# Reecepbcups/celestia-app

Hardware: AMD Instinct MI355X
Metric: ODS→EDS+DAH blocks/sec at k=128 (1/8 GPU); achieved HBM GB/s (higher is better)
Workload: dtype u8; 1 GPU; k128_block_batch: da.ExtendShares+NewDataAvailabilityHeader on 128 independent k=128 blocks per GPU per step (configs[1] per block, batched as configs[2]); k=128, parallelism=blocks x1

## Files before the change

### celestia-app_amd/csrc/cda_internal.h

```cpp
#pragma once
#include <hip/hip_runtime.h>
#include <stddef.h>
#include <stdint.h>

#include "../../include/cda.h"

#define CDA_SHARE 512
#define CDA_REC_WORDS 24
#define CDA_REC_BYTES 96

#ifndef CDA_TEST_HOOKS
#define CDA_TEST_HOOKS 0
#endif
#if CDA_TEST_HOOKS
#define CDA_AB_ENV(name) getenv(name)
#else
#define CDA_AB_ENV(name) ((const char*)nullptr)
#endif

namespace cda {

struct LeoTables {
  int bits;
  unsigned order, modulus;
  const uint16_t* exp_t;
  const uint16_t* log_t;
  const uint16_t* skew;
};
const LeoTables& leo_tables(int bits);
uint64_t leo8_colbits(unsigned log_m);
void leo16_colbits(unsigned log_m, uint16_t out[16]);

struct RsJob {
  const uint8_t* src;
  long long src_blk, src_cw, src_sh;
  uint8_t* dst;
  long long dst_blk, dst_cw, dst_sh;
  uint8_t* cpy;
  long long cpy_blk, cpy_cw, cpy_sh;
  int k;
  int cw_per_blk;
  int nblk;
  int shard_len;
};

int rs_init_device_tables(int device);
int rs16_init_device_tables(int device);
int rs_decode_init_device_tables(int device);
int launch_rs_decode(uint8_t* d_base, const long long* d_off, const long long* d_stride, const uint8_t* d_present,
                     int ncw, int k, int shard_len, hipStream_t s);
int launch_rs_encode8(const RsJob& job, hipStream_t s);
bool rs8_reg_batched(const RsJob& job);
int launch_rs_encode8_pair(const RsJob& ja, const RsJob& jb, bool remap, hipStream_t s);
int launch_q0_copy(const uint8_t* d_ods, uint8_t* d_eds, int k, int nblocks, int max_wgs, hipStream_t s);
int launch_rs_encode16(const RsJob& job, hipStream_t s);
bool rs16_reg_eligible(const RsJob& j);
const char* rs16_diag_tag();
const char* rs8_diag_tag();
int rs16_reg_init(int device);
int launch_rs_encode16_reg(const RsJob& j, const uint16_t* d_cpoly, hipStream_t s);
int launch_leaf_hash(const uint8_t* d_eds, void* d_leaf_nodes, unsigned long long* d_status, int k, int nblocks,
                     hipStream_t s, const uint8_t* d_ods = nullptr);
int launch_nmt_level(const void* d_in, void* d_out, bool from_leaves, int k, int nblocks, int level, hipStream_t s);
int launch_nmt_trees(const void* d_leaves, void* d_levels, void* d_roots, int k, int nblocks, hipStream_t s,
                     void* prof_ctx, bool l1_quads = true);
int launch_dah(const void* d_roots, void* d_dah, int n_roots_total, int nblocks, hipStream_t s);
int launch_dah_tree(const void* d_roots, void* d_dah, void* d_nodes_out, int n_roots_total, hipStream_t s);
int launch_dah_wide(const void* d_roots, void* d_dah, unsigned* d_done, void* d_digests, int n, int nblocks,
                    hipStream_t s);
int launch_trees_lds(const void* d_leaves, void* d_roots, void* d_dah, unsigned* d_done, void* d_digests, int k,
                     int nblocks, hipStream_t s);
int launch_axis_leaf(const uint8_t* d_leaves, int n, uint64_t square_size, uint64_t axis_index, void* d_nodes,
                     unsigned long long* d_status, hipStream_t s);
int launch_level_generic(const void* d_in, void* d_out, int n_in, hipStream_t s);
constexpr int kAxisRootsMaxLeaves = 1024;
int launch_axis_roots(const uint8_t* d_leaves, long long tree_stride, int n, uint64_t square_size,
                      const unsigned long long* d_axis_idx, int ntrees, void* d_roots, unsigned long long* d_status,
                      hipStream_t s);
int launch_axes_roots(const uint8_t* d_eds, int k, const int* d_axes, int axis0, int ntrees, int leaf_off, int nleaves,
                      void* d_nodes, void* d_scratch, void* d_roots, unsigned long long* d_status, hipStream_t s);
int launch_nmt_fold(void* d_nodes, void* d_scratch, void* d_roots, int ntrees, int log2n, hipStream_t s);
int launch_parity_compare(const uint8_t* d_eds, int k, const int* d_axes, int naxes, const uint8_t* d_par,
                          unsigned* d_flags, hipStream_t s);
int launch_axes_verify(const uint8_t* d_eds, int k, const int* d_axes, int ntrees, const uint8_t* d_want_rows,
                       const uint8_t* d_want_cols, unsigned* d_flag, unsigned base, bool per_tree, hipStream_t s);
int launch_roots_check(const void* d_recs, const unsigned long long* d_status, const int* d_axes, int n,
                       const uint8_t* d_want_rows, const uint8_t* d_want_cols, unsigned* d_flag, unsigned base,
                       hipStream_t s);

struct BlobDesc {
  unsigned long long data_off;
  uint32_t len;
  uint32_t share_off;
  uint32_t nshares;
  uint32_t width;
  uint8_t ns[32];
};
int launch_blob_shares(const BlobDesc* d_desc, int nblobs, const uint8_t* d_data, uint32_t total, uint8_t* d_shares,
                       hipStream_t s);
int launch_blob_leaves(const uint8_t* d_shares, uint32_t total, void* d_recs, hipStream_t s);
int launch_blob_mountain_level(const BlobDesc* d_desc, int nblobs, void* d_recs, uint32_t total, int level,
                               hipStream_t s);
int launch_pack_tree_level(const void* d_recs, void* d_out, int log2w, int h, bool col, uint32_t t0, uint32_t nt,
                           uint32_t off_h, hipStream_t s);
int launch_merkle_sets(const void* d_recs, const uint32_t* d_idx, const uint32_t* d_off, int nsets, int max_set,
                       void* d_out, void* d_nodes_out, hipStream_t s);

int launch_scatter_cell_runs(const void* d_compact, void* d_dst, const uint32_t* d_dst_cell, const uint32_t* d_pre,
                             int nruns, uint32_t ncells, hipStream_t s, bool same_layout = false);
int launch_build_ods(const cda_share_segment* d_segs, int nseg, const uint8_t* d_data, const uint32_t* d_reserved,
                     uint32_t nshares, void* d_ods, hipStream_t s);

struct TreeSpec {
  const void* leaves;
  unsigned long long t_stride, i_stride;
  uint32_t ntrees;
  bool tree_fastest;
  void* scratch;
  void* roots;
  unsigned long long r_stride;
};

inline int raise_dynamic_lds(const void* kernel, size_t bytes) {
  if (bytes <= 64 * 1024) return 0;
  return hipFuncSetAttribute(kernel, hipFuncAttributeMaxDynamicSharedMemorySize, (int)bytes) == hipSuccess ? 0 : -1;
}

struct SubtreeLaunch {
  int M, log2n_out;
};
inline SubtreeLaunch subtree_launch(int L, int l_in) {
  const int rest = L - l_in;
  const int M = rest == 3 ? 3 : (rest < 2 ? rest : 2);
  return {M, rest - M};
}
inline unsigned long long levels_before(unsigned long long trees, int L, int l) {
// ... 16 lines not shown
```

### celestia-app_amd/csrc/ctx.h

```cpp
#pragma once
#include <hip/hip_runtime.h>

#include <map>
#include <mutex>
#include <string>
#include <thread>
#include <vector>

#include "arena.h"
#include "cda_internal.h"
#include "mixed_route.h"

namespace cda {
struct AxisQueue;
struct Stager;
struct Consensus;
}
struct cda_square;

struct cda_ctx {
  int device = 0;
  std::vector<int> local_cpus;
  std::recursive_mutex mu;
  hipStream_t stream = nullptr;
  bool repair_overlap = true;
  bool repair_fused_verify = true;
  bool repair_early = true;
  bool l1_quads = true;
  int rs_sched = 2;
  size_t rs_min_ods_bytes = (size_t)256 << 20;
  bool rs_q3_cols = false;
  bool rs_pair_remap = false;
  int q0_copy_wgs = 64;
  hipStream_t q0_stream = nullptr;
  hipEvent_t q0_fork_ev = nullptr, q0_join_ev = nullptr;
  hipStream_t aux_stream = nullptr;
  hipEvent_t ws_event = nullptr, sync_ev = nullptr;
  bool ws_pending = false;
  static constexpr int kSlots = 3;
  hipStream_t h2d_stream = nullptr, d2h_stream = nullptr;
  hipEvent_t ev_h2d[kSlots] = {}, ev_comp[kSlots] = {}, ev_d2h[kSlots] = {};
  static constexpr int kJoin = 2;
  hipEvent_t fork_ev = nullptr, join_ev[kJoin] = {};
  std::string last_err;
  struct Buf {
    void* p = nullptr;
    size_t cap = 0;
  };
  Buf ods, eds, leaf, scratch, roots, dah, status, plan, payload;
  Buf done;
  Buf nodes;
  std::vector<cda_square*> squares;
  Buf sp_ods, sp_R, sp_LR, sp_S, sp_C, sp_LC, sp_scratch, sp_meta, sp_gather;
  hipEvent_t sp_ev[2] = {};
  Buf rdesc, rstage;
  Buf rcompact, rruns;
  cda::Stager* st_in = nullptr;
  cda::Stager* st_out = nullptr;
  int staging = 3;
  cda::Consensus* cons = nullptr;
  bool consensus = true;
  int cons_in = 0, cons_out = 0, cons_stg_mib = -1, copy_threads = 7;
  bool cons_trace = false;
  bool huge_pages = false;
  int mixed_small_max = cda::kMixedSmallMaxDefault;
  cda::AxisQueue* axq = nullptr;
  bool prof = false;
  struct Pending {
    std::string name;
    hipEvent_t a, b;
  };
  std::vector<Pending> pending;
  std::vector<hipEvent_t> event_pool;
  std::map<std::string, std::pair<double, long long>> prof_acc;
};

namespace cda {

constexpr uint32_t kMaxDeviceK = 512;
constexpr int kLdsTreesMax = 512;

bool dev_ok(cda_ctx* c, hipError_t e, const char* what);
int ensure(cda_ctx* c, cda_ctx::Buf& b, size_t bytes);
void flush_profile(cda_ctx* c);
struct Stage {
  cda_ctx* c;
  hipStream_t s;
  Arena ar;
  bool ok = true;
  template <class T>
  T* stage(const T* src, size_t count) {
    T* at = ar.take<T>(count);
    if (ok && at && count && !dev_ok(c, hipMemcpyAsync(at, src, count * sizeof(T), hipMemcpyHostToDevice, s), "H2D"))
      ok = false;
    return at;
  }
};
template <class Lay>
size_t staged_bytes(Lay& lay) {
  Stage measure{nullptr, nullptr, Arena()};
  lay(measure);
  return measure.ar.used();
}
inline bool copy_any(cda_ctx* c, void* dst, const void* src, size_t n, hipStream_t s) {
  return n == 0 || dev_ok(c, hipMemcpyAsync(dst, src, n, hipMemcpyDefault, s), "copy");
}
inline int verdicts_back(cda_ctx* c, void* dst, const void* d_src, size_t n, hipStream_t s) {
  if (!dev_ok(c, hipMemcpyAsync(dst, d_src, n, hipMemcpyDeviceToHost, s), "D2H") ||
      !dev_ok(c, hipStreamSynchronize(s), "sync"))
    return CDA_E_DEVICE;
  flush_profile(c);
  return CDA_OK;
}
int ilog2i(uint32_t v);
bool is_pow2(uint64_t v);
// ... 111 lines not shown
```

### celestia-app_amd/csrc/engine.cpp

```cpp
#include <hip/hip_runtime.h>

#include <algorithm>
#include <chrono>
#include <cmath>
#include <cstdlib>
#include <cstdio>
#include <cstring>
#include <map>
#include <mutex>
#include <string>
#include <system_error>
#include <thread>
#include <vector>

#include "ctx.h"
#include "small_square.h"

namespace cda {

ProfScope::ProfScope(void* c, const char* n, hipStream_t s) : ctx(c), name(n), stream(s), a(nullptr), b(nullptr) {
  cda_ctx* x = static_cast<cda_ctx*>(ctx);
  if (!x || !x->prof) return;
  auto get = [&]() {
    hipEvent_t e;
// ... 121 lines not shown
  j.cpy_cw = j.dst_cw;
  j.cpy_sh = S;
  j.k = (int)k;
  j.cw_per_blk = (int)k;
  j.nblk = (int)nblocks;
  j.shard_len = CDA_SHARE;
  return j;
}

RsJob cols_job(uint32_t k, uint32_t nblocks, uint8_t* d_eds) {
  const uint32_t w = 2 * k;
  const long long S = CDA_SHARE;
  RsJob j{};
  j.src = d_eds;
  j.src_blk = (long long)w * w * S;
  j.src_cw = S;
  j.src_sh = (long long)w * S;
  j.dst = d_eds + (size_t)k * w * S;
  j.dst_blk = j.src_blk;
  j.dst_cw = S;
  j.dst_sh = (long long)w * S;
  j.cpy = nullptr;
  j.k = (int)k;
  j.cw_per_blk = (int)w;
  j.nblk = (int)nblocks;
  j.shard_len = CDA_SHARE;
  return j;
}

int enqueue_rs(cda_ctx* c, uint32_t k, uint32_t nblocks, const uint8_t* d_ods, uint8_t* d_eds, hipStream_t s) {
  {
    const RsJob j = rows_job(k, nblocks, d_ods, d_eds);
    ProfScope ps(c, 2 * k <= 256 ? "rs_encode8_rows" : "rs_encode16_rows", s);
    const int lr = 2 * k <= 256 ? launch_rs_encode8(j, s) : launch_rs_encode16(j, s);
    if (lr) return lr == -2 ? CDA_E_UNSUPPORTED : CDA_E_DEVICE;
  }
  {
    const RsJob j = cols_job(k, nblocks, d_eds);
    ProfScope ps(c, 2 * k <= 256 ? "rs_encode8_cols" : "rs_encode16_cols", s);
    const int lr = 2 * k <= 256 ? launch_rs_encode8(j, s) : launch_rs_encode16(j, s);
    if (lr) return lr == -2 ? CDA_E_UNSUPPORTED : CDA_E_DEVICE;
  }
  return CDA_OK;
}

static RsJob quadrant_job(uint32_t k, uint32_t nblocks, const uint8_t* src, long long src_blk, long long src_pitch,
                          uint8_t* dst, bool by_cols) {
  const uint32_t w = 2 * k;
  const long long S = CDA_SHARE;
  RsJob j{};
  j.src = src;
  j.src_blk = src_blk;
  j.src_cw = by_cols ? S : src_pitch;
  j.src_sh = by_cols ? src_pitch : S;
  j.dst = dst;
  j.dst_blk = (long long)w * w * S;
  j.dst_cw = by_cols ? S : (long long)w * S;
  j.dst_sh = by_cols ? (long long)w * S : S;
  j.k = (int)k;
  j.cw_per_blk = (int)k;
  j.nblk = (int)nblocks;
  j.shard_len = CDA_SHARE;
  return j;
}

static bool rs_from_ods(const cda_ctx* c, uint32_t k, uint32_t nblocks, const uint8_t* d_ods, const uint8_t* d_eds,
                        hipStream_t s) {
  const uintptr_t ods_bytes = (uintptr_t)nblocks * k * k * CDA_SHARE;
  if (c->rs_sched == 0 || s == c->stream || ods_bytes < c->rs_min_ods_bytes) return false;
  if (2 * k > 256 || !is_pow2(k) || !rs8_reg_batched(rows_job(k, nblocks, d_ods, const_cast<uint8_t*>(d_eds))))
    return false;
  const uintptr_t o = (uintptr_t)d_ods, e = (uintptr_t)d_eds, ods_b = (uintptr_t)nblocks * k * k * CDA_SHARE;
  return o + ods_b <= e || e + 4 * ods_b <= o;
}

static int enqueue_rs_from_ods(cda_ctx* c, uint32_t k, uint32_t nblocks, const uint8_t* d_ods, uint8_t* d_eds,
                               hipStream_t s) {
  const long long S = CDA_SHARE, w = 2 * k, eds_blk = w * w * S;
  uint8_t *q1 = d_eds + k * S, *q2 = d_eds + k * w * S, *q3 = q2 + k * S;
  {
    const RsJob ja = quadrant_job(k, nblocks, d_ods, (long long)k * k * S, k * S, q1, false);
    const RsJob jb = quadrant_job(k, nblocks, d_ods, (long long)k * k * S, k * S, q2, true);
    ProfScope ps(c, "rs_encode8_rows", s);
    const int lr = launch_rs_encode8_pair(ja, jb, c->rs_pair_remap, s);
    if (lr) return lr == -2 ? CDA_E_UNSUPPORTED : CDA_E_DEVICE;
  }
  {
    const RsJob j = c->rs_q3_cols ? quadrant_job(k, nblocks, q1, eds_blk, w * S, q3, true)
                                  : quadrant_job(k, nblocks, q2, eds_blk, w * S, q3, false);
    ProfScope ps(c, "rs_encode8_cols", s);
    const int lr = launch_rs_encode8(j, s);
    if (lr) return lr == -2 ? CDA_E_UNSUPPORTED : CDA_E_DEVICE;
  }
  return CDA_OK;
}

static bool lds_trees_path(uint32_t k, uint32_t nblocks) {
  static const int lds_trees = CDA_AB_ENV("CDA_TREES_LDS") ? atoi(CDA_AB_ENV("CDA_TREES_LDS")) : kLdsTreesMax;
  return (size_t)nblocks * 4 * k <= (size_t)lds_trees && 2 * k <= 256;
}

int prepare_trees(cda_ctx* c, uint32_t k, uint32_t nblocks, hipStream_t s) {
  if (!lds_trees_path(k, nblocks) && 2 * k < 1024) return CDA_OK;
  const size_t cnt_b = ((size_t)nblocks * 4 + 255) & ~(size_t)255, need = cnt_b + (size_t)nblocks * 4 * k * 32;
  if (c->done.cap >= need) return CDA_OK;
  int rc = ensure(c, c->done, std::max<size_t>(need, 64 * 1024));
  if (rc) return rc;
  return dev_ok(c, hipMemsetAsync(c->done.p, 0, c->done.cap, s), "hipMemsetAsync") ? CDA_OK : CDA_E_DEVICE;
}

int enqueue_trees(cda_ctx* c, uint32_t k, uint32_t nblocks, void* d_roots, void* d_dah, hipStream_t s, size_t rec_off) {
  const uint32_t w = 2 * k;
  if (lds_trees_path(k, nblocks)) {
    const size_t cnt_b = ((size_t)nblocks * 4 + 255) & ~(size_t)255;
    if (int rc = prepare_trees(c, k, nblocks, s)) return rc;
    ProfScope ps(c, "trees_lds", s);
    const int lr = launch_trees_lds((uint8_t*)c->leaf.p + rec_off * CDA_REC_BYTES, d_roots, d_dah,
                                    (unsigned*)c->done.p, (uint8_t*)c->done.p + cnt_b, (int)k, (int)nblocks, s);
    if (lr) return lr == -2 ? CDA_E_UNSUPPORTED : CDA_E_DEVICE;
    return CDA_OK;
  }
  const int lr0 = launch_nmt_trees((uint8_t*)c->leaf.p + rec_off * CDA_REC_BYTES,
                                   (uint8_t*)c->scratch.p + 2 * rec_off * CDA_REC_BYTES, d_roots, (int)k, (int)nblocks, s,
                                   c, c->l1_quads);
  if (lr0) return lr0 == -2 ? CDA_E_UNSUPPORTED : CDA_E_DEVICE;
  if (w < 1024) {
    ProfScope ps(c, "dah", s);
    const int lr = launch_dah(d_roots, d_dah, (int)(2 * w), (int)nblocks, s);
    if (lr) return lr == -2 ? CDA_E_UNSUPPORTED : CDA_E_DEVICE;
  } else {
    const size_t cnt_b = ((size_t)nblocks * 4 + 255) & ~(size_t)255;
    if (int rc = prepare_trees(c, k, nblocks, s)) return rc;
    ProfScope ps(c, "dah", s);
    const int lr = launch_dah_wide(d_roots, d_dah, (unsigned*)c->done.p, (uint8_t*)c->done.p + cnt_b, (int)(2 * w),
                                   (int)nblocks, s);
    if (lr) return lr == -2 ? CDA_E_UNSUPPORTED : CDA_E_DEVICE;
  }
  return CDA_OK;
}

int enqueue_commit(cda_ctx* c, uint32_t k, uint32_t nblocks, const uint8_t* d_eds, void* d_roots, void* d_dah,
                   unsigned long long* d_status, hipStream_t s, size_t rec_off, bool init_status) {
  if (init_status && !dev_ok(c, hipMemsetAsync(d_status, 0xFF, (size_t)nblocks * 8, s), "hipMemsetAsync"))
    return CDA_E_DEVICE;
  {
    ProfScope ps(c, "leaf_hash", s);
    if (launch_leaf_hash(d_eds, bufs0(c, rec_off), d_status, (int)k, (int)nblocks, s)) return CDA_E_DEVICE;
  }
  return enqueue_trees(c, k, nblocks, d_roots, d_dah, s, rec_off);
}

int enqueue_pipeline(cda_ctx* c, uint32_t k, uint32_t nblocks, const uint8_t* d_ods, uint8_t* d_eds, void* d_roots,
                     void* d_dah, unsigned long long* d_status, hipStream_t s) {
  const uint32_t w = 2 * k;
  const size_t cells = (size_t)nblocks * w * w;
  int rc = ensure(c, c->leaf, cells * CDA_REC_BYTES);
  if (rc) return rc;
  rc = ensure(c, c->scratch, 2 * cells * CDA_REC_BYTES);
  if (rc) return rc;
  if (!dev_ok(c, hipMemsetAsync(d_status, 0xFF, (size_t)nblocks * 8, s), "hipMemsetAsync")) return CDA_E_DEVICE;
  if (!rs_from_ods(c, k, nblocks, d_ods, d_eds, s)) {
    if ((rc = enqueue_rs(c, k, nblocks, d_ods, d_eds, s))) return rc;
    return enqueue_commit(c, k, nblocks, d_eds, d_roots, d_dah, d_status, s, 0, false);
  }
  if ((rc = enqueue_rs_from_ods(c, k, nblocks, d_ods, d_eds, s))) return rc;
  const bool side = c->rs_sched == 2;
  const hipStream_t q0s = c->q0_stream;
  if (side && (!dev_ok(c, hipEventRecord(c->q0_fork_ev, s), "hipEventRecord") ||
               !dev_ok(c, hipStreamWaitEvent(q0s, c->q0_fork_ev, 0), "hipStreamWaitEvent")))
    return CDA_E_DEVICE;
  if (const int lr = launch_q0_copy(d_ods, d_eds, (int)k, (int)nblocks, side ? c->q0_copy_wgs : 0,
                                    side ? q0s : s))
    return lr == -2 ? CDA_E_UNSUPPORTED : CDA_E_DEVICE;
  if (side && !dev_ok(c, hipEventRecord(c->q0_join_ev, q0s), "hipEventRecord")) {
    (void)hipStreamSynchronize(q0s);
    return CDA_E_DEVICE;
  }
  {
    ProfScope ps(c, "leaf_hash", s);
    if (launch_leaf_hash(d_eds, bufs0(c, 0), d_status, (int)k, (int)nblocks, s, side ? d_ods : nullptr))
      rc = CDA_E_DEVICE;
  }
  if (!rc) rc = enqueue_trees(c, k, nblocks, d_roots, d_dah, s, 0);
  if (side && !dev_ok(c, hipStreamWaitEvent(s, c->q0_join_ev, 0), "hipStreamWaitEvent")) {
    (void)hipStreamSynchronize(q0s);
    return CDA_E_DEVICE;
  }
  return rc;
}

void pack_roots(const uint8_t* recs, uint32_t n, uint8_t* out) {
  for (uint32_t i = 0; i < n; i++) memcpy(out + (size_t)i * CDA_NODE_SIZE, recs + (size_t)i * CDA_REC_BYTES, CDA_NODE_SIZE);
}

int map_status(uint64_t st, int block, cda_err_info* err) {
  if (st == ~0ull) return CDA_OK;
  set_err(err, CDA_E_NS_ORDER, (int)(st >> 40), (int)((st >> 20) & 0xFFFFF), (int)(st & 0xFFFFF), block);
  return CDA_E_NS_ORDER;
}


}

extern "C" {

int cda_init(int device, cda_ctx** out) {
  CDA_API_TRY
  if (!out) return CDA_E_ARG;
  *out = nullptr;
  int n = 0;
  if (hipGetDeviceCount(&n) != hipSuccess || device < 0 || device >= n) return CDA_E_DEVICE;
  if (hipSetDevice(device) != hipSuccess) return CDA_E_DEVICE;
  cda_ctx* c = new cda_ctx();
  struct Owner {
    cda_ctx* c;
    ~Owner() {
      if (c) cda_free(c);
    }
  } own{c};
  c->device = device;
  const char* fail = nullptr;
  if (hipStreamCreateWithFlags(&c->stream, hipStreamNonBlocking) != hipSuccess) fail = "stream";
  else if (rs_init_device_tables(device)) fail = "rs8 tables";
  else if (rs16_init_device_tables(device)) fail = "rs16 tables";
  else if (rs_decode_init_device_tables(device)) fail = "decode tables";
  else if (small_square_init(device)) fail = "small-square tables";
  if (fail) {
    fprintf(stderr, "cda_init: %s initialisation failed: %s\n", fail, hipGetErrorString(hipGetLastError()));
    return CDA_E_DEVICE;
  }
  if (const char* e = CDA_AB_ENV("CDA_REPAIR_OVERLAP")) c->repair_overlap = atoi(e) != 0;
  if (const char* e = CDA_AB_ENV("CDA_REPAIR_FUSED")) c->repair_fused_verify = atoi(e) != 0;
  if (const char* e = CDA_AB_ENV("CDA_REPAIR_EARLY")) c->repair_early = atoi(e) != 0;
  if (const char* e = CDA_AB_ENV("CDA_L1_QUADS")) c->l1_quads = atoi(e) != 0;
  if (const char* e = CDA_AB_ENV("CDA_STAGING")) c->staging = atoi(e) & 3;
  if (const char* e = CDA_AB_ENV("CDA_CONSENSUS")) c->consensus = atoi(e) != 0;
  if (const char* e = CDA_AB_ENV("CDA_CONS_IN")) c->cons_in = std::max(0, std::min(2, atoi(e)));
  if (const char* e = CDA_AB_ENV("CDA_CONS_OUT")) c->cons_out = atoi(e) == 2 ? 2 : 0;
  if (const char* e = CDA_AB_ENV("CDA_CONS_STG")) c->cons_stg_mib = std::max(0, atoi(e));
  if (const char* e = getenv("CDA_COPY_THREADS")) c->copy_threads = std::max(1, std::min(64, atoi(e)));
  if (const char* e = CDA_AB_ENV("CDA_HUGE_PAGES")) c->huge_pages = atoi(e) != 0;
  c->cons_trace = CDA_AB_ENV("CDA_CONS_TRACE") != nullptr;
  if (const char* e = CDA_AB_ENV("CDA_RS_SCHED")) c->rs_sched = std::max(0, std::min(2, atoi(e)));
  if (const char* e = CDA_AB_ENV("CDA_RS_MIN_ODS_MIB")) c->rs_min_ods_bytes = (size_t)std::max(0, atoi(e)) << 20;
  if (const char* e = CDA_AB_ENV("CDA_RS_Q3")) c->rs_q3_cols = e[0] == 'c';
  if (const char* e = CDA_AB_ENV("CDA_RS_PAIR_REMAP")) c->rs_pair_remap = atoi(e) != 0;
  if (const char* e = CDA_AB_ENV("CDA_Q0_COPY_WGS")) c->q0_copy_wgs = std::max(0, atoi(e));
  find_local_cpus(c);
  bool ok = ensure_pipeline(c) == CDA_OK &&
            hipStreamCreateWithFlags(&c->aux_stream, hipStreamNonBlocking) == hipSuccess &&
            hipStreamCreateWithFlags(&c->q0_stream, hipStreamNonBlocking) == hipSuccess &&
            hipEventCreateWithFlags(&c->q0_fork_ev, hipEventDisableTiming) == hipSuccess &&
            hipEventCreateWithFlags(&c->q0_join_ev, hipEventDisableTiming) == hipSuccess &&
            hipEventCreateWithFlags(&c->fork_ev, hipEventDisableTiming) == hipSuccess &&
            hipEventCreateWithFlags(&c->ws_event, hipEventDisableTiming) == hipSuccess &&
            hipEventCreateWithFlags(&c->sync_ev, hipEventDisableTiming) == hipSuccess;
  for (int i = 0; i < cda_ctx::kJoin && ok; i++)
    ok = hipEventCreateWithFlags(&c->join_ev[i], hipEventDisableTiming) == hipSuccess;
  if (!ok) return CDA_E_DEVICE;
  own.c = nullptr;
  *out = c;
  return CDA_OK;
  CDA_API_CATCH(nullptr)
}

void cda_free(cda_ctx* c) {
  if (!c) return;
  try {
    Lock l(c);
    (void)hipStreamSynchronize(c->stream);
    flush_profile(c);
    release_squares(c);
    for (auto* b : {&c->ods, &c->eds, &c->leaf, &c->scratch, &c->roots, &c->dah, &c->status, &c->plan, &c->payload,
                    &c->rdesc, &c->rcompact, &c->rruns, &c->done, &c->nodes, &c->sp_ods, &c->sp_R, &c->sp_LR, &c->sp_S, &c->sp_C, &c->sp_LC, &c->sp_scratch,
                    &c->sp_meta, &c->sp_gather})
      if (b->p) (void)hipFree(b->p);
    for (auto e : c->sp_ev)
      if (e) (void)hipEventDestroy(e);
    if (c->rstage.p) (void)hipHostFree(c->rstage.p);
    for (auto e : c->event_pool) (void)hipEventDestroy(e);
    for (int i = 0; i < cda_ctx::kJoin; i++)
      if (c->join_ev[i]) (void)hipEventDestroy(c->join_ev[i]);
    free_consensus(c);
    free_axisq(c);
    free_pipeline(c);
    free_staging(c);
    if (c->aux_stream) (void)hipStreamDestroy(c->aux_stream);
    if (c->q0_stream) (void)hipStreamDestroy(c->q0_stream);
    if (c->q0_fork_ev) (void)hipEventDestroy(c->q0_fork_ev);
    if (c->q0_join_ev) (void)hipEventDestroy(c->q0_join_ev);
    if (c->fork_ev) (void)hipEventDestroy(c->fork_ev);
    if (c->ws_event) (void)hipEventDestroy(c->ws_event);
    if (c->sync_ev) (void)hipEventDestroy(c->sync_ev);
    if (c->stream) (void)hipStreamDestroy(c->stream);
  } catch (...) {
  }
  delete c;
}

const char* cda_strerror(int code) {
  switch (code) {
    case CDA_OK: return "ok";
    case CDA_E_NOT_POW2: return "number of shares is not a power of 2";
    case CDA_E_NOT_SQUARE: return "number of chunks must be a square number";
    case CDA_E_SHARD_SIZE: return "chunk size must be a multiple of 64 bytes";
    case CDA_E_NS_SHORT: return "data is too short to contain namespace ID";
    case CDA_E_NS_ORDER: return "pushed data has smaller namespace than previous (invalid push order)";
    case CDA_E_TOO_FEW: return "too few shards given";
    case CDA_E_UNREPAIRABLE: return "failed to solve data square";
    case CDA_E_BYZANTINE: return "byzantine data";
    case CDA_E_ARG: return "invalid argument";
    case CDA_E_DEVICE: return "device error";
    case CDA_E_PUSH_PAST: return "pushed past predetermined square size";
    case CDA_E_UNSUPPORTED: return "unsupported configuration";
    case CDA_E_SHARE_VERSION: return "unsupported share version";
    case CDA_E_BLOB_SIZE: return "cannot use zero blob size";
    case CDA_E_NOMEM: return "out of host memory";
    case CDA_E_INTERNAL: return "internal error (exception caught at the C ABI)";
    default: return "unknown error";
  }
}

const char* cda_last_device_error(cda_ctx* c) { return c ? c->last_err.c_str() : ""; }

const char* cda_build_info(void) {
  static const std::string info = [] {
    std::string d;
    for (const char* t : {rs8_diag_tag(), rs16_diag_tag(), CDA_TEST_HOOKS ? "test_hooks" : ""})
      if (*t) d += (d.empty() ? "" : ",") + std::string(t);
// ... 331 lines not shown
```

### celestia-app_amd/csrc/rs_kernels.hip

```cpp
#include <hip/hip_runtime.h>
#include <stdint.h>
#include <stdlib.h>

#include <vector>

#include "cda_internal.h"
#include "codec_shape.h"
#include "gf8_const.h"
#include "gf_slice.h"
#include "rs8_lds_dev.h"

namespace cda {

__constant__ uint16_t c_skew8[256];
__constant__ unsigned long long c_col8[256];

struct Rs8ConstTables {
  __device__ __forceinline__ unsigned skew(int i) const { return c_skew8[i]; }
  __device__ __forceinline__ unsigned long long col(unsigned log_m) const { return c_col8[log_m]; }
};

struct Rs8Args {
  const uint8_t* src;
  long long src_blk, src_cw, src_sh;
  uint8_t* dst;
  long long dst_blk, dst_cw, dst_sh;
  uint8_t* cpy;
  long long cpy_blk, cpy_cw, cpy_sh;
  int k, m, log2m, cw_per_blk, U, log2U, slices;
  int lat;
};

__global__ void __launch_bounds__(256) rs_encode8_kernel(Rs8Args a) {
  extern __shared__ __attribute__((aligned(16))) uint32_t st[];
  const int U = a.U;
  int wg = blockIdx.x;
  const int slice = wg % a.slices;
  wg /= a.slices;
  const int cw = wg % a.cw_per_blk;
  const int blk = wg / a.cw_per_blk;
  const long long byte_off = (long long)slice * U * 32;
  const uint8_t* src = a.src + blk * a.src_blk + cw * a.src_cw + byte_off;
  uint8_t* dst = a.dst + blk * a.dst_blk + cw * a.dst_cw + byte_off;
  uint8_t* cpy = a.cpy ? a.cpy + blk * a.cpy_blk + cw * a.cpy_cw + byte_off : nullptr;

  unsigned long long* s_cb = nullptr;
  if (a.lat) {
    s_cb = reinterpret_cast<unsigned long long*>(st + 8 * (a.m << a.log2U));
    for (int i = threadIdx.x; i < 256; i += blockDim.x) s_cb[i] = c_col8[c_skew8[i]];
  }
  const int items = a.m << a.log2U;
  if (items <= 2 * (int)blockDim.x) {
    uint4 v[2][2];
#pragma unroll
    for (int it = 0; it < 2; it++) {
      const int e = threadIdx.x + it * blockDim.x, s = e >> a.log2U, u = e & (U - 1);
      if (e < items && s < a.k) {
        const uint4* p = reinterpret_cast<const uint4*>(src + s * a.src_sh + u * 32);
        v[it][0] = p[0];
        v[it][1] = p[1];
      }
    }
#pragma unroll
    for (int it = 0; it < 2; it++) {
      const int e = threadIdx.x + it * blockDim.x, s = e >> a.log2U, u = e & (U - 1);
      if (e >= items) continue;
      uint32_t w[8];
      if (s < a.k) {
        if (cpy) {
          uint4* q = reinterpret_cast<uint4*>(cpy + s * a.cpy_sh + u * 32);
          q[0] = v[it][0];
          q[1] = v[it][1];
        }
        w[0] = v[it][0].x; w[1] = v[it][0].y; w[2] = v[it][0].z; w[3] = v[it][0].w;
        w[4] = v[it][1].x; w[5] = v[it][1].y; w[6] = v[it][1].z; w[7] = v[it][1].w;
        bitslice8(w);
      } else {
#pragma unroll
        for (int j = 0; j < 8; j++) w[j] = 0;
      }
#pragma unroll
      for (int j = 0; j < 8; j++) st[j * items + lds_sw(s * U + u)] = w[j];
    }
  }
  for (int e = threadIdx.x; items > 2 * (int)blockDim.x && e < items; e += blockDim.x) {
    const int s = e >> a.log2U, u = e & (U - 1);
    uint32_t w[8];
    if (s < a.k) {
      const uint4* p = reinterpret_cast<const uint4*>(src + s * a.src_sh + u * 32);
      uint4 v0 = p[0], v1 = p[1];
      if (cpy) {
        uint4* q = reinterpret_cast<uint4*>(cpy + s * a.cpy_sh + u * 32);
        q[0] = v0;
// ... 151 lines not shown
  constexpr int x = x2_of(W, 0, R, 1);
  constexpr unsigned c = kCpoly8.v[INVERSE ? (M - 1 + x + 1) : x];
  {
    uint32_t T[8];
    if constexpr (INVERSE) {
#pragma unroll
      for (int j = 0; j < 8; j++) T[j] = lane_pair_xor(E[R][j]);
    } else {
      lane_pair_xor8(T, E[R]);
    }
    if constexpr (INVERSE) {
      if constexpr (c != 0u) gf8_muladd_cantor<c>(E[R], T);
#pragma unroll
      for (int j = 0; j < 8; j++) E[R][j] = __builtin_amdgcn_bitop3_b32(lm, E[R][j], T[j], 0xCA);
    } else {
      uint32_t S[8];
#pragma unroll
      for (int j = 0; j < 8; j++) {
        S[j] = __builtin_amdgcn_bitop3_b32(E[R][j], T[j], lm, 0x78);
        E[R][j] = __builtin_amdgcn_bitop3_b32(lm, E[R][j], T[j], 0xCA);
      }
      if constexpr (c != 0u) gf8_muladd_cantor<c>(E[R], S);
    }
#pragma unroll
    for (int j = 0; j < 8; j++) asm volatile("" : "+v"(E[R][j]));
  }
  __builtin_amdgcn_sched_barrier(0);
}

template <bool INVERSE, int M, int W>
__device__ __forceinline__ void layer_d0_w(uint32_t (&E)[8][8], uint32_t lm) {
  d0_w<INVERSE, M, W, 0>(E, lm);
  d0_w<INVERSE, M, W, 1>(E, lm);
  d0_w<INVERSE, M, W, 2>(E, lm);
  d0_w<INVERSE, M, W, 3>(E, lm);
  d0_w<INVERSE, M, W, 4>(E, lm);
  d0_w<INVERSE, M, W, 5>(E, lm);
  d0_w<INVERSE, M, W, 6>(E, lm);
  d0_w<INVERSE, M, W, 7>(E, lm);
}

template <int L, int W>
__device__ __forceinline__ void p1_w(uint32_t (&E)[8][8], uint32_t lm) {
  constexpr int M = 1 << L;
  layer_d0_w<true, M, W>(E, lm);
  layer_w<true, M, W, 1>(E);
  if constexpr (L > 2) layer_w<true, M, W, 2>(E);
  if constexpr (L > 3) layer_w<true, M, W, 3>(E);
}

template <int L, int W>
__device__ __forceinline__ void p3_w(uint32_t (&E)[8][8], uint32_t lm) {
  constexpr int M = 1 << L, F2 = L - 3;
  if constexpr (F2 - 1 >= 3) layer_w<false, M, W, 3>(E);
  if constexpr (F2 - 1 >= 2) layer_w<false, M, W, 2>(E);
  if constexpr (F2 - 1 >= 1) layer_w<false, M, W, 1>(E);
  layer_d0_w<false, M, W>(E, lm);
}

template <int M>
__device__ __forceinline__ void exchange2(uint32_t (&E)[8][8], uint4* xbuf, int w, int sw, int li, int f_from,
                                          int f_to) {
#pragma unroll
  for (int h = 0; h < 2; h++) {
#pragma unroll
    for (int r = 0; r < 8; r++) {
      const int x = x2_of(w, sw, r, f_from);
      xbuf[x * 32 + li] = make_uint4(E[r][4 * h], E[r][4 * h + 1], E[r][4 * h + 2], E[r][4 * h + 3]);
    }
    __syncthreads();
#pragma unroll
    for (int r = 0; r < 8; r++) {
      const int x = x2_of(w, sw, r, f_to);
      const uint4 v = xbuf[x * 32 + li];
      E[r][4 * h] = v.x;
      E[r][4 * h + 1] = v.y;
      E[r][4 * h + 2] = v.z;
      E[r][4 * h + 3] = v.w;
    }
    __syncthreads();
  }
}

template <int L, int WC>
__device__ __forceinline__ void rs_g2_impl(const Rs8RegArgs& a, int wg, uint4* xbuf, int w) {
  constexpr int M = 1 << L;
  const int lane = threadIdx.x & 63;
  const int sw = lane & 1, li = lane >> 1;
  const int u = li & 15, cwi = li >> 4;
  uint32_t lm = sw ? 0u : ~0u;
  asm volatile("" : "+v"(lm));
  const int slice = wg % a.slices;
  wg /= a.slices;
  const int grp = wg % a.groups_per_blk;
  const int blk = wg / a.groups_per_blk;
  const int cw = grp * 2 + cwi;
  const long long off = (long long)slice * 512 + u * 16;
  const uint8_t* src = a.src + blk * a.src_blk + cw * a.src_cw + off;
  uint8_t* dst = a.dst + blk * a.dst_blk + cw * a.dst_cw + off;
  uint8_t* cpy = a.cpy ? a.cpy + blk * a.cpy_blk + cw * a.cpy_cw + off : nullptr;

  uint32_t E[8][8];
  const SliceMasks km = slice_masks();
  constexpr int wv = WC;
#pragma unroll
  for (int r = 0; r < 8; r++) {
    const int x = x2_of(wv, sw, r, 1), x0 = x2_of(wv, 0, r, 1);
    if (x0 < a.k) {
      const uint4* p = reinterpret_cast<const uint4*>(src + x * a.src_sh);
      const uint4 v0 = p[0], v1 = p[16];
      if (cpy) {
        uint4* q = reinterpret_cast<uint4*>(cpy + x * a.cpy_sh);
        q[0] = v0;
        q[16] = v1;
      }
      E[r][0] = v0.x; E[r][1] = v0.y; E[r][2] = v0.z; E[r][3] = v0.w;
      E[r][4] = v1.x; E[r][5] = v1.y; E[r][6] = v1.z; E[r][7] = v1.w;
      bitslice8(E[r], km);
    } else {
#pragma unroll
      for (int j = 0; j < 8; j++) E[r][j] = 0;
    }
  }
  constexpr int F2 = L - 3;
#ifndef CDA_RS8_DIAG_NOCOMPUTE
  p1_w<L, WC>(E, lm);
  if (L > 4) exchange2<M>(E, xbuf, WC, sw, li, 1, F2);
  p2_layers<L, (F2 > 1 ? F2 : 1), 4, true>(E);
  if (L > 4) exchange2<M>(E, xbuf, WC, sw, li, F2, 1);
  p3_w<L, WC>(E, lm);
#else
  (void)lm;
  (void)F2;
#endif
  const SliceMasks ko = slice_masks();
#pragma unroll
  for (int r = 0; r < 8; r++) {
    const int x = x2_of(wv, sw, r, 1), x0 = x2_of(wv, 0, r, 1);
    if (x0 < a.k) {
      uint32_t v[8];
#pragma unroll
      for (int j = 0; j < 8; j++) v[j] = E[r][j];
      bitslice8(v, ko);
      uint4* q = reinterpret_cast<uint4*>(dst + x * a.dst_sh);
      q[0] = make_uint4(v[0], v[1], v[2], v[3]);
      q[16] = make_uint4(v[4], v[5], v[6], v[7]);
    }
  }
}

template <int L, int W>
__device__ __forceinline__ void rs_g2_select(const Rs8RegArgs& a, int wg, uint4* xbuf, int w) {
  if constexpr (W < (1 << (L - 4))) {
    if (w == W)
      rs_g2_impl<L, W>(a, wg, xbuf, w);
    else
      rs_g2_select<L, W + 1>(a, wg, xbuf, w);
  }
}

template <int L>
__device__ __forceinline__ void rs_g2_body(const Rs8RegArgs& a, int wg, uint4* xbuf) {
  const int w = __builtin_amdgcn_readfirstlane(threadIdx.x >> 6) & ((1 << (L - 4)) - 1);
  rs_g2_select<L, 0>(a, wg, xbuf, w);
}

template <int L>
__global__ void __launch_bounds__(64 << (L - 4), 4) rs_encode8_g2_kernel(Rs8RegArgs a, Rs8RegArgs a2) {
  extern __shared__ __attribute__((aligned(16))) uint4 xbuf[];
  const unsigned g = gridDim.x, b = blockIdx.x;
  int wg = (a.remap && (g % 8u) == 0) ? (int)((b % 8u) * (g / 8u) + b / 8u) : (int)b;
  bool second = false;
  if (a.pair) {
    const int gpb = a.groups_per_blk, blk = wg / (2 * gpb), rem = wg - blk * 2 * gpb;
    second = rem >= gpb;
    wg = blk * gpb + (second ? rem - gpb : rem);
  }
  Rs8RegArgs j = a;
  j.src = second ? a2.src : a.src;
  j.src_blk = second ? a2.src_blk : a.src_blk;
  j.src_cw = second ? a2.src_cw : a.src_cw;
  j.src_sh = second ? a2.src_sh : a.src_sh;
  j.dst = second ? a2.dst : a.dst;
  j.dst_blk = second ? a2.dst_blk : a.dst_blk;
  j.dst_cw = second ? a2.dst_cw : a.dst_cw;
  j.dst_sh = second ? a2.dst_sh : a.dst_sh;
  rs_g2_body<L>(j, wg, xbuf);
}

__global__ void __launch_bounds__(256) rs_q0_copy_kernel(const uint4* __restrict__ ods, uint4* __restrict__ eds,
                                                         int log2row, int log2k, unsigned long long total) {
  for (unsigned long long chunk = blockIdx.x; chunk * 1024 < total; chunk += gridDim.x) {
    const unsigned long long i0 = chunk * 1024 + threadIdx.x;
    uint4 v[4];
#pragma unroll
    for (int q = 0; q < 4; q++)
      if (i0 + q * 256 < total) v[q] = ods[i0 + q * 256];
#pragma unroll
    for (int q = 0; q < 4; q++) {
      const unsigned long long i = i0 + q * 256;
      if (i >= total) continue;
      const unsigned long long row = i >> log2row, blk = row >> log2k, r = row & ((1ull << log2k) - 1);
      eds[((((blk << (log2k + 1)) + r) << (log2row + 1))) + (i & ((1ull << log2row) - 1))] = v[q];
    }
  }
}

static Rs8RegArgs reg_args(const RsJob& j);

int rs_init_device_tables(int device) {
  (void)device;
  const LeoTables& t = leo_tables(8);
  uint16_t skew[256];
  unsigned long long col[256];
  for (int i = 0; i < 255; i++) skew[i] = t.skew[i];
  skew[255] = 255;
  for (unsigned l = 0; l < 256; l++) col[l] = leo8_colbits(l);
  if (hipMemcpyToSymbol(HIP_SYMBOL(c_skew8), skew, sizeof skew) != hipSuccess) return -1;
  if (hipMemcpyToSymbol(HIP_SYMBOL(c_col8), col, sizeof col) != hipSuccess) return -1;
  uint8_t apow[255];
  unsigned st = 1;
  for (int i = 0; i < 255; i++) {
    apow[i] = (uint8_t)st;
    st <<= 1;
    if (st & 0x100) st ^= 0x11D;
  }
  uint8_t cpoly[256];
  for (int i = 0; i < 256; i++) cpoly[i] = skew[i] >= 255 ? 0 : apow[skew[i]];
  for (int i = 0; i < 256; i++)
    if (cpoly[i] != kCpoly8.v[i]) return -1;
  if (hipFuncSetAttribute((const void*)rs_encode8_kernel, hipFuncAttributeMaxDynamicSharedMemorySize,
                          kRsEncode8MaxLds) != hipSuccess)
    return -1;
  const void* g2k[4] = {(const void*)rs_encode8_g2_kernel<4>, (const void*)rs_encode8_g2_kernel<5>,
                        (const void*)rs_encode8_g2_kernel<6>, (const void*)rs_encode8_g2_kernel<7>};
  for (auto f : g2k)
    if (hipFuncSetAttribute(f, hipFuncAttributeMaxDynamicSharedMemorySize, 64 * 1024) != hipSuccess) return -1;

  return 0;
}

static int ilog2(int v) {
  int l = 0;
  while ((1 << l) < v) l++;
  return l;
}

static Rs8RegArgs reg_args(const RsJob& j) {
  Rs8RegArgs r{};
  r.src = j.src;
  r.src_blk = j.src_blk;
  r.src_cw = j.src_cw;
  r.src_sh = j.src_sh;
  r.dst = j.dst;
  r.dst_blk = j.dst_blk;
  r.dst_cw = j.dst_cw;
  r.dst_sh = j.dst_sh;
  r.cpy = j.cpy;
  r.cpy_blk = j.cpy_blk;
  r.cpy_cw = j.cpy_cw;
  r.cpy_sh = j.cpy_sh;
  r.k = j.k;
  r.groups_per_blk = j.cw_per_blk / 2;
  r.slices = j.shard_len / 512;
  r.remap = j.src_sh == j.shard_len;
  return r;
}

static int rs8_lat_u() {
  static const int lat_u = [] {
    const char* e = CDA_AB_ENV("CDA_RS8_LAT_U");
    const int v = e ? atoi(e) : kRs8LatU;
    return (v == 1 || v == 2 || v == 4 || v == 8 || v == 16) ? v : 0;
  }();
  return lat_u;
}

bool rs8_reg_batched(const RsJob& j) {
  return rs8_reg_batched_shape(j.k, j.shard_len, j.cw_per_blk, j.nblk, rs8_lat_u());
}

static int launch_g2(int L, long long grid, const Rs8RegArgs& r, const Rs8RegArgs& r2, hipStream_t s) {
  if (grid <= 0 || grid > 0x7FFFFFFF) return -2;
  const size_t lds = rs8_reg_lds_bytes(L);
  const dim3 block(64 << (L - 4));
  switch (L) {
    case 4: hipLaunchKernelGGL(rs_encode8_g2_kernel<4>, dim3((unsigned)grid), block, lds, s, r, r2); break;
    case 5: hipLaunchKernelGGL(rs_encode8_g2_kernel<5>, dim3((unsigned)grid), block, lds, s, r, r2); break;
    case 6: hipLaunchKernelGGL(rs_encode8_g2_kernel<6>, dim3((unsigned)grid), block, lds, s, r, r2); break;
    default: hipLaunchKernelGGL(rs_encode8_g2_kernel<7>, dim3((unsigned)grid), block, lds, s, r, r2); break;
  }
  return hipGetLastError() == hipSuccess ? 0 : -1;
}

int launch_rs_encode8_pair(const RsJob& ja, const RsJob& jb, bool remap, hipStream_t s) {
  if (!rs8_reg_batched(ja) || !rs8_reg_batched(jb) || ja.shard_len != 512 || jb.shard_len != 512 || ja.k != jb.k ||
      ja.cw_per_blk != jb.cw_per_blk || ja.nblk != jb.nblk || ja.cpy || jb.cpy)
    return -2;
  Rs8RegArgs r = reg_args(ja);
  const Rs8RegArgs r2 = reg_args(jb);
  r.remap = remap;
  r.pair = 1;
  return launch_g2(ilog2(ja.k), 2ll * ja.nblk * r.groups_per_blk, r, r2, s);
}

int launch_q0_copy(const uint8_t* d_ods, uint8_t* d_eds, int k, int nblocks, int max_wgs, hipStream_t s) {
  if (k < 1 || (k & (k - 1)) || nblocks < 1) return -2;
  const int log2k = ilog2(k);
  const unsigned long long total = (unsigned long long)nblocks * k * k * (CDA_SHARE / 16);
  unsigned long long grid = (total + 1023) / 1024;
  if (max_wgs > 0 && grid > (unsigned long long)max_wgs) grid = max_wgs;
  if (grid > 0x7FFFFFFFull) return -2;
  hipLaunchKernelGGL(rs_q0_copy_kernel, dim3((unsigned)grid), dim3(256), 0, s, (const uint4*)d_ods, (uint4*)d_eds,
                     log2k + 5, log2k, total);
  return hipGetLastError() == hipSuccess ? 0 : -1;
}

int launch_rs_encode8(const RsJob& j, hipStream_t s) {
  const RsEncode8Shape sh = rs_encode8_shape(j.k, j.shard_len, j.cw_per_blk, j.nblk, rs8_lat_u());
  if (!sh.ok) return -2;
  if (sh.reg) {
    const Rs8RegArgs r = reg_args(j);
    return launch_g2(sh.log2m, sh.grid, r, r, s);
  }
  Rs8Args a;
  a.src = j.src;
  a.src_blk = j.src_blk;
  a.src_cw = j.src_cw;
  a.src_sh = j.src_sh;
  a.dst = j.dst;
  a.dst_blk = j.dst_blk;
  a.dst_cw = j.dst_cw;
  a.dst_sh = j.dst_sh;
  a.cpy = j.cpy;
  a.cpy_blk = j.cpy_blk;
  a.cpy_cw = j.cpy_cw;
  a.cpy_sh = j.cpy_sh;
  a.k = j.k;
  a.log2m = sh.log2m;
  a.m = sh.m;
  a.cw_per_blk = j.cw_per_blk;
  a.U = sh.U;
  a.log2U = sh.log2U;
  a.slices = sh.slices;
  a.lat = sh.lat;
  hipLaunchKernelGGL(rs_encode8_kernel, dim3((unsigned)sh.grid), dim3(256), sh.lds_bytes, s, a);
  return hipGetLastError() == hipSuccess ? 0 : -1;
}

constexpr uint16_t kPhi16[16] = {0x0001, 0xACCA, 0x3C0E, 0x163E, 0xC582, 0xED2E, 0x914C, 0x4012,
                                 0x6C98, 0x10D8, 0x6A72, 0xB900, 0xFDB8, 0xFB34, 0xFF38, 0x991E};
constexpr uint16_t kPhiInv16[16] = {0x0001, 0x4690, 0x65D8, 0x62D0, 0x5734, 0x45F0, 0x53B8, 0x1E38,
                                    0x7CAE, 0x4E38, 0x6708, 0xC25C, 0x7A64, 0x9EAC, 0x1124, 0x523A};

__device__ __forceinline__ void apply16(uint32_t (&v)[16], const uint16_t (&cols)[16]) {
  uint32_t o[16];
#pragma unroll
  for (int i = 0; i < 16; i++) {
    uint32_t acc = 0;
#pragma unroll
    for (int j = 0; j < 16; j++)
      if ((cols[j] >> i) & 1) acc ^= v[j];
    o[i] = acc;
  }
#pragma unroll
  for (int i = 0; i < 16; i++) v[i] = o[i];
}

__device__ __forceinline__ void xtime16(uint32_t (&T)[16]) {
  const uint32_t t = T[15];
#pragma unroll
  for (int i = 15; i > 0; i--) T[i] = T[i - 1];
  T[0] = t;
  T[2] ^= t;
  T[3] ^= t;
  T[5] ^= t;
}

__device__ __forceinline__ void gf16_muladd_uniform(uint32_t (&X)[16], const uint32_t (&Y)[16], unsigned c) {
  uint32_t T[16];
#pragma unroll
  for (int j = 0; j < 16; j++) T[j] = Y[j];
#pragma unroll
  for (int i = 0; i < 16; i++) {
    if (c & (1u << i)) {
// ... 227 lines not shown
```

Measured before the change: 20420 blocks/s.

## Add sliced, XCD-aware work mapping for paired RS8 row encode kernel

Adds a sliced variant of the paired GF(2^8) register encode kernel. Each workgroup handles 256-byte slices across 4 codewords instead of 512-byte slices across 2, and blocks are mapped so each slice group's workgroups spread round-robin across the 8 XCDs. Parity stores in this path use inline global_store_dwordx4 with the sc1 cache-policy bit. The path is on by default with an env override; the aim is better L2 locality and spread across XCDs for the row-pair encode, at the cost of more kernel instantiations and hand-written store assembly.

```diff
diff --git a/celestia-app_amd/csrc/cda_internal.h b/celestia-app_amd/csrc/cda_internal.h
--- a/celestia-app_amd/csrc/cda_internal.h
+++ b/celestia-app_amd/csrc/cda_internal.h
@@ -51,7 +51,7 @@
                      int ncw, int k, int shard_len, hipStream_t s);
 int launch_rs_encode8(const RsJob& job, hipStream_t s);
 bool rs8_reg_batched(const RsJob& job);
-int launch_rs_encode8_pair(const RsJob& ja, const RsJob& jb, bool remap, hipStream_t s);
+int launch_rs_encode8_pair(const RsJob& ja, const RsJob& jb, bool remap, bool sliced, hipStream_t s);
 int launch_q0_copy(const uint8_t* d_ods, uint8_t* d_eds, int k, int nblocks, int max_wgs, hipStream_t s);
 int launch_rs_encode16(const RsJob& job, hipStream_t s);
 bool rs16_reg_eligible(const RsJob& j);
diff --git a/celestia-app_amd/csrc/ctx.h b/celestia-app_amd/csrc/ctx.h
--- a/celestia-app_amd/csrc/ctx.h
+++ b/celestia-app_amd/csrc/ctx.h
@@ -31,6 +31,7 @@
   size_t rs_min_ods_bytes = (size_t)256 << 20;
   bool rs_q3_cols = false;
   bool rs_pair_remap = false;
+  bool rs_a_sliced = true;
   int q0_copy_wgs = 64;
   hipStream_t q0_stream = nullptr;
   hipEvent_t q0_fork_ev = nullptr, q0_join_ev = nullptr;
diff --git a/celestia-app_amd/csrc/engine.cpp b/celestia-app_amd/csrc/engine.cpp
--- a/celestia-app_amd/csrc/engine.cpp
+++ b/celestia-app_amd/csrc/engine.cpp
@@ -227,7 +227,7 @@
     const RsJob ja = quadrant_job(k, nblocks, d_ods, (long long)k * k * S, k * S, q1, false);
     const RsJob jb = quadrant_job(k, nblocks, d_ods, (long long)k * k * S, k * S, q2, true);
     ProfScope ps(c, "rs_encode8_rows", s);
-    const int lr = launch_rs_encode8_pair(ja, jb, c->rs_pair_remap, s);
+    const int lr = launch_rs_encode8_pair(ja, jb, c->rs_pair_remap, c->rs_a_sliced, s);
     if (lr) return lr == -2 ? CDA_E_UNSUPPORTED : CDA_E_DEVICE;
   }
   {
@@ -390,6 +390,7 @@
   if (const char* e = CDA_AB_ENV("CDA_RS_MIN_ODS_MIB")) c->rs_min_ods_bytes = (size_t)std::max(0, atoi(e)) << 20;
   if (const char* e = CDA_AB_ENV("CDA_RS_Q3")) c->rs_q3_cols = e[0] == 'c';
   if (const char* e = CDA_AB_ENV("CDA_RS_PAIR_REMAP")) c->rs_pair_remap = atoi(e) != 0;
+  if (const char* e = CDA_AB_ENV("CDA_RS_A_SLICED")) c->rs_a_sliced = atoi(e) != 0;
   if (const char* e = CDA_AB_ENV("CDA_Q0_COPY_WGS")) c->q0_copy_wgs = std::max(0, atoi(e));
   find_local_cpus(c);
   bool ok = ensure_pipeline(c) == CDA_OK &&
diff --git a/celestia-app_amd/csrc/rs_kernels.hip b/celestia-app_amd/csrc/rs_kernels.hip
--- a/celestia-app_amd/csrc/rs_kernels.hip
+++ b/celestia-app_amd/csrc/rs_kernels.hip
@@ -9,6 +9,7 @@
 #include "gf8_const.h"
 #include "gf_slice.h"
 #include "rs8_lds_dev.h"
+#include "rs_slice_map.h"
 
 namespace cda {
 
@@ -326,20 +327,31 @@
   }
 }
 
-template <int L, int WC>
+typedef uint32_t rs_u32x4 __attribute__((ext_vector_type(4)));
+template <int H>
+__device__ __forceinline__ void rs_store2_sc1(uint4* q, const uint32_t (&v)[8]) {
+  const rs_u32x4 lo = {v[0], v[1], v[2], v[3]}, hi = {v[4], v[5], v[6], v[7]};
+  asm volatile("global_store_dwordx4 %0, %1, off sc1\n\tglobal_store_dwordx4 %0, %2, off offset:%3 sc1\n\ts_nop 1"
+               :
+               : "v"(q), "v"(lo), "v"(hi), "n"(H * 16)
+               : "memory");
+}
+
+template <int L, int WC, bool SL>
 __device__ __forceinline__ void rs_g2_impl(const Rs8RegArgs& a, int wg, uint4* xbuf, int w) {
   constexpr int M = 1 << L;
   const int lane = threadIdx.x & 63;
   const int sw = lane & 1, li = lane >> 1;
-  const int u = li & 15, cwi = li >> 4;
+  const int u = SL ? li & (kRsSliceBytes / 32 - 1) : li & 15, cwi = SL ? li / (kRsSliceBytes / 32) : li >> 4;
   uint32_t lm = sw ? 0u : ~0u;
   asm volatile("" : "+v"(lm));
   const int slice = wg % a.slices;
   wg /= a.slices;
   const int grp = wg % a.groups_per_blk;
   const int blk = wg / a.groups_per_blk;
-  const int cw = grp * 2 + cwi;
-  const long long off = (long long)slice * 512 + u * 16;
+  const int cw = grp * (SL ? kRsSliceCw : 2) + cwi;
+  constexpr int H = SL ? kRsSliceBytes / 32 : 16;
+  const long long off = (long long)slice * (SL ? kRsSliceBytes : 512) + u * 16;
   const uint8_t* src = a.src + blk * a.src_blk + cw * a.src_cw + off;
   uint8_t* dst = a.dst + blk * a.dst_blk + cw * a.dst_cw + off;
   uint8_t* cpy = a.cpy ? a.cpy + blk * a.cpy_blk + cw * a.cpy_cw + off : nullptr;
@@ -352,11 +364,11 @@
     const int x = x2_of(wv, sw, r, 1), x0 = x2_of(wv, 0, r, 1);
     if (x0 < a.k) {
       const uint4* p = reinterpret_cast<const uint4*>(src + x * a.src_sh);
-      const uint4 v0 = p[0], v1 = p[16];
+      const uint4 v0 = p[0], v1 = p[H];
       if (cpy) {
         uint4* q = reinterpret_cast<uint4*>(cpy + x * a.cpy_sh);
         q[0] = v0;
-        q[16] = v1;
+        q[H] = v1;
       }
       E[r][0] = v0.x; E[r][1] = v0.y; E[r][2] = v0.z; E[r][3] = v0.w;
       E[r][4] = v1.x; E[r][5] = v1.y; E[r][6] = v1.z; E[r][7] = v1.w;
@@ -387,38 +399,49 @@
       for (int j = 0; j < 8; j++) v[j] = E[r][j];
       bitslice8(v, ko);
       uint4* q = reinterpret_cast<uint4*>(dst + x * a.dst_sh);
-      q[0] = make_uint4(v[0], v[1], v[2], v[3]);
-      q[16] = make_uint4(v[4], v[5], v[6], v[7]);
-    }
-  }
-}
-
-template <int L, int W>
+      if (SL) {
+        rs_store2_sc1<H>(q, v);
+      } else {
+        q[0] = make_uint4(v[0], v[1], v[2], v[3]);
+        q[H] = make_uint4(v[4], v[5], v[6], v[7]);
+      }
+    }
+  }
+}
+
+template <int L, int W, bool SL>
 __device__ __forceinline__ void rs_g2_select(const Rs8RegArgs& a, int wg, uint4* xbuf, int w) {
   if constexpr (W < (1 << (L - 4))) {
     if (w == W)
-      rs_g2_impl<L, W>(a, wg, xbuf, w);
+      rs_g2_impl<L, W, SL>(a, wg, xbuf, w);
     else
-      rs_g2_select<L, W + 1>(a, wg, xbuf, w);
-  }
-}
-
-template <int L>
+      rs_g2_select<L, W + 1, SL>(a, wg, xbuf, w);
+  }
+}
+
+template <int L, bool SL>
 __device__ __forceinline__ void rs_g2_body(const Rs8RegArgs& a, int wg, uint4* xbuf) {
   const int w = __builtin_amdgcn_readfirstlane(threadIdx.x >> 6) & ((1 << (L - 4)) - 1);
-  rs_g2_select<L, 0>(a, wg, xbuf, w);
-}
-
-template <int L>
+  rs_g2_select<L, 0, SL>(a, wg, xbuf, w);
+}
+
+template <int L, bool SL = false>
 __global__ void __launch_bounds__(64 << (L - 4), 4) rs_encode8_g2_kernel(Rs8RegArgs a, Rs8RegArgs a2) {
   extern __shared__ __attribute__((aligned(16))) uint4 xbuf[];
-  const unsigned g = gridDim.x, b = blockIdx.x;
-  int wg = (a.remap && (g % 8u) == 0) ? (int)((b % 8u) * (g / 8u) + b / 8u) : (int)b;
+  int wg;
   bool second = false;
-  if (a.pair) {
-    const int gpb = a.groups_per_blk, blk = wg / (2 * gpb), rem = wg - blk * 2 * gpb;
-    second = rem >= gpb;
-    wg = blk * gpb + (second ? rem - gpb : rem);
+  if constexpr (SL) {
+    const RsSliceWork sw = rs_slice_work(blockIdx.x, a.k, (int)(gridDim.x / (2u * kRsSlices * a.groups_per_blk)));
+    second = sw.job != 0;
+    wg = (sw.blk * a.groups_per_blk + sw.grp) * kRsSlices + sw.slice;
+  } else {
+    const unsigned g = gridDim.x, b = blockIdx.x;
+    wg = (a.remap && (g % 8u) == 0) ? (int)((b % 8u) * (g / 8u) + b / 8u) : (int)b;
+    if (a.pair) {
+      const int gpb = a.groups_per_blk, blk = wg / (2 * gpb), rem = wg - blk * 2 * gpb;
+      second = rem >= gpb;
+      wg = blk * gpb + (second ? rem - gpb : rem);
+    }
   }
   Rs8RegArgs j = a;
   j.src = second ? a2.src : a.src;
@@ -429,7 +452,7 @@
   j.dst_blk = second ? a2.dst_blk : a.dst_blk;
   j.dst_cw = second ? a2.dst_cw : a.dst_cw;
   j.dst_sh = second ? a2.dst_sh : a.dst_sh;
-  rs_g2_body<L>(j, wg, xbuf);
+  rs_g2_body<L, SL>(j, wg, xbuf);
 }
 
 __global__ void __launch_bounds__(256) rs_q0_copy_kernel(const uint4* __restrict__ ods, uint4* __restrict__ eds,
@@ -476,8 +499,10 @@
   if (hipFuncSetAttribute((const void*)rs_encode8_kernel, hipFuncAttributeMaxDynamicSharedMemorySize,
                           kRsEncode8MaxLds) != hipSuccess)
     return -1;
-  const void* g2k[4] = {(const void*)rs_encode8_g2_kernel<4>, (const void*)rs_encode8_g2_kernel<5>,
-                        (const void*)rs_encode8_g2_kernel<6>, (const void*)rs_encode8_g2_kernel<7>};
+  const void* g2k[8] = {(const void*)rs_encode8_g2_kernel<4>,       (const void*)rs_encode8_g2_kernel<5>,
+                        (const void*)rs_encode8_g2_kernel<6>,       (const void*)rs_encode8_g2_kernel<7>,
+                        (const void*)rs_encode8_g2_kernel<4, true>, (const void*)rs_encode8_g2_kernel<5, true>,
+                        (const void*)rs_encode8_g2_kernel<6, true>, (const void*)rs_encode8_g2_kernel<7, true>};
   for (auto f : g2k)
     if (hipFuncSetAttribute(f, hipFuncAttributeMaxDynamicSharedMemorySize, 64 * 1024) != hipSuccess) return -1;
 
@@ -524,10 +549,20 @@
   return rs8_reg_batched_shape(j.k, j.shard_len, j.cw_per_blk, j.nblk, rs8_lat_u());
 }
 
-static int launch_g2(int L, long long grid, const Rs8RegArgs& r, const Rs8RegArgs& r2, hipStream_t s) {
+static int launch_g2(int L, long long grid, const Rs8RegArgs& r, const Rs8RegArgs& r2, hipStream_t s,
+                     bool sliced = false) {
   if (grid <= 0 || grid > 0x7FFFFFFF) return -2;
   const size_t lds = rs8_reg_lds_bytes(L);
   const dim3 block(64 << (L - 4));
+  if (sliced) {
+    switch (L) {
+      case 4: hipLaunchKernelGGL((rs_encode8_g2_kernel<4, true>), dim3((unsigned)grid), block, lds, s, r, r2); break;
+      case 5: hipLaunchKernelGGL((rs_encode8_g2_kernel<5, true>), dim3((unsigned)grid), block, lds, s, r, r2); break;
+      case 6: hipLaunchKernelGGL((rs_encode8_g2_kernel<6, true>), dim3((unsigned)grid), block, lds, s, r, r2); break;
+      default: hipLaunchKernelGGL((rs_encode8_g2_kernel<7, true>), dim3((unsigned)grid), block, lds, s, r, r2); break;
+    }
+    return hipGetLastError() == hipSuccess ? 0 : -1;
+  }
   switch (L) {
     case 4: hipLaunchKernelGGL(rs_encode8_g2_kernel<4>, dim3((unsigned)grid), block, lds, s, r, r2); break;
     case 5: hipLaunchKernelGGL(rs_encode8_g2_kernel<5>, dim3((unsigned)grid), block, lds, s, r, r2); break;
@@ -537,14 +572,20 @@
   return hipGetLastError() == hipSuccess ? 0 : -1;
 }
 
-int launch_rs_encode8_pair(const RsJob& ja, const RsJob& jb, bool remap, hipStream_t s) {
+int launch_rs_encode8_pair(const RsJob& ja, const RsJob& jb, bool remap, bool sliced, hipStream_t s) {
   if (!rs8_reg_batched(ja) || !rs8_reg_batched(jb) || ja.shard_len != 512 || jb.shard_len != 512 || ja.k != jb.k ||
       ja.cw_per_blk != jb.cw_per_blk || ja.nblk != jb.nblk || ja.cpy || jb.cpy)
     return -2;
   Rs8RegArgs r = reg_args(ja);
   const Rs8RegArgs r2 = reg_args(jb);
+  r.pair = 1;
+  if (sliced && rs_slice_ok(ja.k) && ja.cw_per_blk == ja.k) {
+    r.remap = 0;
+    r.groups_per_blk = ja.k / kRsSliceCw;
+    r.slices = kRsSlices;
+    return launch_g2(ilog2(ja.k), rs_slice_grid(ja.k, ja.nblk), r, r2, s, true);
+  }
   r.remap = remap;
-  r.pair = 1;
   return launch_g2(ilog2(ja.k), 2ll * ja.nblk * r.groups_per_blk, r, r2, s);
 }
 
diff --git a/celestia-app_amd/csrc/rs_slice_map.h b/celestia-app_amd/csrc/rs_slice_map.h
--- /dev/null
+++ b/celestia-app_amd/csrc/rs_slice_map.h
@@ -0,0 +1,41 @@
+#pragma once
+
+namespace cda {
+
+constexpr int kRsSliceBytes = 256;
+constexpr int kRsSlices = 512 / kRsSliceBytes;
+constexpr int kRsSliceCw = 1024 / kRsSliceBytes;
+constexpr int kRsXcds = 8;
+
+struct RsSliceWork {
+  int blk, slice;
+  int job;
+  int grp;
+};
+
+constexpr bool rs_slice_ok(int k) { return k >= 16 && k % 8 == 0; }
+
+constexpr long long rs_slice_grid(int k, int nblk) { return (long long)nblk * kRsSlices * 2 * (k / kRsSliceCw); }
+
+constexpr RsSliceWork rs_slice_work(unsigned b, int k, int nblk) {
+  const unsigned M = 2 * ((unsigned)k / kRsSliceCw);
+  const unsigned groups = (unsigned)nblk * kRsSlices, rounds = groups / kRsXcds;
+  const unsigned full = rounds * kRsXcds * M;
+  unsigned group = 0, member = 0;
+  if (b < full) {
+    const unsigned round = b / (kRsXcds * M), rem = b - round * (kRsXcds * M);
+    group = round * kRsXcds + rem % kRsXcds;
+    member = rem / kRsXcds;
+  } else {
+    group = rounds * kRsXcds + (b - full) / M;
+    member = (b - full) % M;
+  }
+  RsSliceWork r{};
+  r.blk = (int)(group / kRsSlices);
+  r.slice = (int)(group % kRsSlices);
+  r.job = (int)(member & 1u);
+  r.grp = (int)(member >> 1);
+  return r;
+}
+
+}
```

Result: no change. 20600 blocks/s, median of 6 (+0.9%).
